# lnkloveating/MediQuery-RAG

Hardware: AMD Instinct MI355X
Metric: queries/s (embed+top-k, k=5, b=256) over 1M×768 corpus; p50 single-query ms (higher is better)
Workload: dtype f32 (exact 3-way bf16 split, fp32 accumulate; exact fp32 top-k)

## Files before the change

mediquery-rag_amd/csrc/encoder.hip:

```cpp
#include <algorithm>
#include <cmath>
#include <cstdlib>
#include <cstring>
#include <memory>
#include <vector>

#include "common.hpp"
#include "gemm_epi.hpp"
#include "gemm_f32.hpp"
#include "gemm_x6p.hpp"

namespace mq {


constexpr int kLnPartW = 96;
constexpr int kLnMaxParts = 8;
struct LnArgs {
  float* stats_out;
  const float* stats_in;
  const float* g;
  const float* b;
  float* xout;
  int ldx;
  int nt;
// ... 94 lines not shown
                                                         const float* __restrict__ W,
                                                         const float* __restrict__ bias,
                                                         const float* __restrict__ resid, int ldr,
                                                         float* __restrict__ out, int ldo, int M,
                                                         int N, int K, LnArgs ln, int rx) {
  __shared__ __attribute__((aligned(16))) float lds[2 * T::STAGE_FLOATS];
  __shared__ float2 ln_st[LN_IN ? 2 * T::BM : 1];
  const int lane = threadIdx.x & 63, wave = __builtin_amdgcn_readfirstlane(threadIdx.x >> 6);
  const int wm = wave / T::WAVES_N, wn = wave % T::WAVES_N;
  const int tiles_n = (N + T::BN - 1) / T::BN, tiles_m = (M + T::BM - 1) / T::BM;
  const int G = gridDim.x, per_xcd = G >> 3;
  const int xslot = (blockIdx.x & 7) * per_xcd + (blockIdx.x >> 3);
  Region rg{0, tiles_m, 0, tiles_n};
  int loc = xslot, wstep = G;
  if (rx > 0) {
    rg = region_of(rx, blockIdx.x & 7, tiles_m, tiles_n);
    loc = blockIdx.x >> 3;
    wstep = per_xcd;
  }
  const int rtiles = rg.rm * rg.rn;
  const int n_tiles = loc < rtiles ? (rtiles - loc + wstep - 1) / wstep : 0;
  const FastDiv tnd(rg.rn);
  auto coords = [&](int i, int& m0, int64_t& n0) {
    const int t = i * wstep + loc;
    const int tr = tnd.div(t);
    m0 = (rg.m_lo + tr) * T::BM;
    n0 = (int64_t)(rg.n_lo + t - tr * rg.rn) * T::BN;
  };
  auto epi = [&](int i, floatx16(&acc)[T::TM][T::TN], float*) {
    int m0;
    int64_t n0l;
    coords(i, m0, n0l);
    const int n0 = (int)n0l;
    if constexpr (EPI == EPI_RESID_STATS) {
      static_assert(T::WN == kLnPartW, "stats partials are per kLnPartW-column wave tile");
      const int wr0 = m0 + wm * T::WM, wc0 = n0 + wn * T::WN;
      const int part = wc0 / T::WN;
      float bv[T::TN];
#pragma unroll
      for (int tn = 0; tn < T::TN; ++tn) bv[tn] = bias[wc0 + tn * 32 + (lane & 31)];
      float rv[T::TM][T::TN][16];
      const bool full = m0 + T::BM <= M;
      const __amdgpu_buffer_rsrc_t ro = __builtin_amdgcn_make_buffer_rsrc(
          (void*)(out + (int64_t)wr0 * ldo + wc0), (short)0, 0x7fffffff, 0x00020000);
      const int ol = (4 * (lane >> 5) * ldo + (lane & 31)) * 4;
      if (full) {
        const __amdgpu_buffer_rsrc_t rr = __builtin_amdgcn_make_buffer_rsrc(
            (void*)(resid + (int64_t)wr0 * ldr + wc0), (short)0, 0x7fffffff, 0x00020000);
        const int rl = (4 * (lane >> 5) * ldr + (lane & 31)) * 4;
#pragma unroll
        for (int tm = 0; tm < T::TM; ++tm)
#pragma unroll
          for (int tn = 0; tn < T::TN; ++tn)
#pragma unroll
            for (int e = 0; e < 16; ++e)
              rv[tm][tn][e] = __uint_as_float(__builtin_amdgcn_raw_buffer_load_b32(
                  rr, rl, (acc_row(tm, e, 0) * ldr + tn * 32) * 4, 0));
      } else {
#pragma unroll
        for (int tm = 0; tm < T::TM; ++tm)
#pragma unroll
          for (int tn = 0; tn < T::TN; ++tn)
#pragma unroll
            for (int e = 0; e < 16; ++e) {
              const int row = min(wr0 + acc_row(tm, e, lane), M - 1);
              rv[tm][tn][e] = resid[(int64_t)row * ldr + wc0 + tn * 32 + (lane & 31)];
// ... 1271 lines not shown
namespace {

struct GemmArgs {
  float* slab;
  size_t slab_floats;
  const float* A;
  int lda;
  const float* W;
  const float* bias;
  const float* resid;
  int ldr;
  float* out;
  int ldo;
  int M, N, K;
  int nt = 0;
  const void* W3 = nullptr;
};

template <class T, int EPI, bool LN_IN = false>
void launch_gemm_t(const GemmArgs& g, int num_cus, hipStream_t s, const LnArgs& ln = LnArgs{}) {
  const int tiles = ((g.M + T::BM - 1) / T::BM) * ((g.N + T::BN - 1) / T::BN);
  const int grid = (std::min(tiles, T::WG_PER_CU * num_cus) + 7) / 8 * 8;
  const int tiles_m = (g.M + T::BM - 1) / T::BM, tiles_n = (g.N + T::BN - 1) / T::BN;
  const int rx = region_pick_rx(tiles_m, tiles_n, (double)T::BM * g.K * 4, (double)T::BN * g.K * 4, grid);
  hipLaunchKernelGGL((gemm_nt_kernel<T, EPI, LN_IN>), dim3(grid), dim3(T::THREADS), 0, s, g.A, g.lda, g.W,
                     g.bias, g.resid, g.ldr, g.out, g.ldo, g.M, g.N, g.K, ln, rx);
}

using GemmBig = F32Tile<2, 2, 2, 2>;
using GemmT96 = F32Tile<4, 1, 1, 3>;
using GemmMid = F32Tile<2, 2, 2, 1>;
using GemmSmall = F32Tile<1, 4, 1, 1>;

using X6Big = F32Tile<2, 2, 2, 2, true>;
using X6T96 = F32Tile<4, 1, 1, 3, true>;
using X6Mid = F32Tile<2, 2, 2, 1, true>;

template <int EPI>
void launch_gemm_tile(const GemmArgs& g, int tile, int num_cus, hipStream_t s) {
  switch (tile) {
    case 0: launch_gemm_t<GemmBig, EPI>(g, num_cus, s); return;
    case 1: launch_gemm_t<GemmT96, EPI>(g, num_cus, s); return;
    case 2: launch_gemm_t<GemmMid, EPI>(g, num_cus, s); return;
    case 5: launch_gemm_t<X6Big, EPI>(g, num_cus, s); return;
    case 6: launch_gemm_t<X6T96, EPI>(g, num_cus, s); return;
    case 7: launch_gemm_t<X6Mid, EPI>(g, num_cus, s); return;
    case 8: launch_gemm_t<F32Tile<4, 2, 1, 3>, EPI>(g, num_cus, s); return;
    case 9: launch_gemm_t<F32Tile<4, 2, 1, 3, true>, EPI>(g, num_cus, s); return;
    default: launch_gemm_t<GemmSmall, EPI>(g, num_cus, s); return;
  }
}

int splitk_factor(const GemmArgs& g, int num_cus, int cap = 16, int tiles_max = 0) {
  if (!g.slab || g.N % 4 != 0) return 0;
  const int64_t tiles = (int64_t)((g.M + 31) / 32) * ((g.N + 127) / 128);
  const int64_t slots = 2 * (int64_t)num_cus;
  if (tiles > (tiles_max > 0 ? tiles_max : num_cus) || g.M > 256) return 0;
  const int slices = g.K / kBK;
  int best = 1;
  for (int s = 1; s <= slices && s <= cap; ++s)
    if (slices % s == 0 && tiles * s <= slots && (size_t)s * g.M * g.N <= g.slab_floats) best = s;
  return best >= 2 ? best : 0;
}

void launch_splitk_gemm(const GemmArgs& g, int S, hipStream_t s) {
  auto go = [&](auto tile) {
    using T = decltype(tile);
    const int tiles = ((g.M + T::BM - 1) / T::BM) * ((g.N + T::BN - 1) / T::BN);
    hipLaunchKernelGGL((gemm_splitk_kernel<T>), dim3(tiles * S), dim3(256), 0, s, g.A, g.lda, g.W, g.M, g.N, g.K,
                       S, g.slab);
  };
  if (g.nt)
    go(F32Tile<1, 4, 1, 1, false, 2, false, 0, true>{});
  else
    go(F32Tile<1, 4, 1, 1>{});
}

template <int EPI>
void launch_splitk(const GemmArgs& g, int S, hipStream_t s) {
  launch_splitk_gemm(g, S, s);
  const int64_t n4 = (int64_t)g.M * g.N / 4;
// ... 980 lines not shown
```

mediquery-rag_amd/csrc/gemm_epi.hpp:

```cpp
#pragma once

#include "gemm_f32.hpp"

namespace mq {

enum Epi { EPI_BIAS = 0, EPI_GELU_ERF = 1, EPI_GELU_TANH = 2, EPI_RESID = 3, EPI_RESID_STATS = 4 };

__device__ __forceinline__ float gelu_erf(float x) {
  const float z = fabsf(x) * 0.70710678118654752f;
  const float t = __builtin_amdgcn_rcpf(fmaf(0.5f, z, 1.0f));
  float p = 0.17087277f;
  p = fmaf(p, t, -0.82215223f);
  p = fmaf(p, t, 1.48851587f);
  p = fmaf(p, t, -1.13520398f);
  p = fmaf(p, t, 0.27886807f);
  p = fmaf(p, t, -0.18628806f);
  p = fmaf(p, t, 0.09678418f);
  p = fmaf(p, t, 0.37409196f);
  p = fmaf(p, t, 1.00002368f);
  p = fmaf(p, t, -1.26551223f);
  const float e = t * __builtin_amdgcn_exp2f(fmaf(-z, z, p) * 1.4426950408889634f);
  return x * (x >= 0.f ? fmaf(-0.5f, e, 1.0f) : 0.5f * e);
}
__device__ __forceinline__ float gelu_tanh(float x) {
// ... 33 lines not shown
    const __amdgpu_buffer_rsrc_t ro = __builtin_amdgcn_make_buffer_rsrc(
        (void*)(out + (int64_t)wr0 * ldo + wc0), (short)0, 0x7fffffff, 0x00020000);
    const int ol = (4 * (lane >> 5) * ldo + (lane & 31)) * 4;
#pragma unroll
    for (int tm = 0; tm < TM; ++tm)
#pragma unroll
      for (int tn = 0; tn < TN; ++tn)
#pragma unroll
        for (int e = 0; e < 16; ++e) {
          float v = epi_apply<EPI>(acc[tm][tn][e] + bv[tn]);
          if constexpr (EPI == EPI_RESID) v += rv[tm][tn][e];
          __builtin_amdgcn_raw_buffer_store_b32(__float_as_uint(v), ro, ol, (acc_row(tm, e, 0) * ldo + tn * 32) * 4, 0);
        }
    return;
  }
#pragma unroll
  for (int tn = 0; tn < TN; ++tn) {
    const int col = wc0 + tn * 32 + (lane & 31);
    if (col >= N) continue;
    const float b = bias[col];
#pragma unroll
    for (int tm = 0; tm < TM; ++tm)
#pragma unroll
      for (int e = 0; e < 16; ++e) {
        const int row = wr0 + acc_row(tm, e, lane);
        if (row >= M) continue;
        float v = epi_apply<EPI>(acc[tm][tn][e] + b);
        if constexpr (EPI == EPI_RESID) v += resid[(int64_t)row * ldr + col];
        out[(int64_t)row * ldo + col] = v;
      }
  }
}

}
```

mediquery-rag_amd/csrc/gemm_f32.hpp:

```cpp
#pragma once

#include "common.hpp"

namespace mq {

constexpr int kBK = 32;
constexpr int kLdsStride = kBK + 4;

typedef __bf16 bf16x8 __attribute__((ext_vector_type(8)));
typedef unsigned uintx4 __attribute__((ext_vector_type(4)));

template <int WAVES_M_, int WAVES_N_, int TM_, int TN_, bool X6_ = false, int PF_ = 2,
          bool BF16_ = false, int BK_ = 0, bool NTB_ = false>
struct F32Tile {
  static constexpr int WAVES_M = WAVES_M_, WAVES_N = WAVES_N_, TM = TM_, TN = TN_;
  static constexpr bool X6 = X6_;
  static constexpr bool NTB = NTB_;
  static constexpr int PF = PF_;
  static constexpr bool BF16 = BF16_;
  static_assert(!(X6 && BF16), "one arithmetic mode");
  static constexpr int WM = TM * 32, WN = TN * 32;
  static constexpr int BM = WAVES_M * WM, BN = WAVES_N * WN;
  static constexpr int THREADS = WAVES_M * WAVES_N * kWave;
  static constexpr int ROWS = BM + BN;
  static constexpr int BK = BK_ ? BK_ : (X6 ? 16 : 32);
  static_assert(BK == 32 || (BK == 16 && !BF16), "slice depth 32, or 16 for the f32 forms");
  static constexpr int F4_PER_ROW = BK / 4;
  static constexpr int ROW_FLOATS = X6 ? 28 : BK + 4;
  static constexpr int TOTAL_F4 = ROWS * F4_PER_ROW;
  static constexpr int LOADS = (TOTAL_F4 + THREADS - 1) / THREADS;
  static constexpr bool PARTIAL = TOTAL_F4 % THREADS != 0;
  static constexpr int STAGE_FLOATS = ROWS * ROW_FLOATS;
  static_assert(THREADS == 256 || THREADS == 512, "4- or 8-wave workgroups");
  static constexpr int WG_PER_CU = THREADS == 256 ? 2 : 1;
  static_assert(BM % 32 == 0 && BN % 32 == 0, "block tile must be a multiple of 32");
  static constexpr bool A_SLOTS = (BM * F4_PER_ROW) % THREADS == 0;
};

__device__ __forceinline__ unsigned pk_bf16(float lo, float hi) {
  unsigned r;
  asm("v_cvt_pk_bf16_f32 %0, %1, %2" : "=v"(r) : "v"(lo), "v"(hi));
  return r;
}
__device__ __forceinline__ float bf16_lo(unsigned p) { return __uint_as_float(p << 16); }
__device__ __forceinline__ float bf16_hi(unsigned p) { return __uint_as_float(p & 0xffff0000u); }

__device__ __forceinline__ void split3(floatx4 x, uint2 (&pl)[3]) {
#pragma unroll
  for (int p = 0; p < 3; ++p) {
    const unsigned a = pk_bf16(x.x, x.y), b = pk_bf16(x.z, x.w);
    pl[p] = make_uint2(a, b);
    if (p < 2) {
      x.x -= bf16_lo(a);
      x.y -= bf16_hi(a);
      x.z -= bf16_lo(b);
      x.w -= bf16_hi(b);
    }
  }
}

template <int V>
struct IC {
  static constexpr int value = V;
};

template <int N, int I = 0, class F>
__device__ __forceinline__ void static_for(F&& f) {
// ... 30 lines not shown
          r[i] = __builtin_bit_cast(floatx4, __builtin_amdgcn_raw_buffer_load_b128(
                                                 rb, min(row - T::BM, blim) * b4 + ch * 16, k0 * 4, T::NTB ? 2 : 0));
      }
      return;
    }
#pragma unroll
    for (int i = 0; i < T::LOADS; ++i) {
      const int f = tid + i * T::THREADS;
      if (T::PARTIAL && i == T::LOADS - 1 && f >= T::TOTAL_F4) break;
      const int row = f / T::F4_PER_ROW, ch = f % T::F4_PER_ROW;
      const float* p;
      const bool a_row = T::A_SLOTS ? i < T::BM * T::F4_PER_ROW / T::THREADS
                                    : f < T::BM * T::F4_PER_ROW;
      if (a_row) {
        p = A + (int64_t)min(m0 + row, M - 1) * lda;
      } else {
        p = B + min(n0 + (int64_t)(row - T::BM), N - 1) * ldb;
      }
      r[i] = *reinterpret_cast<const floatx4*>(p + k0 + ch * 4);
    }
  }

  __device__ __forceinline__ void store(float* stage, int tid) const {
#pragma unroll
    for (int i = 0; i < T::LOADS; ++i) {
      const int f = tid + i * T::THREADS;
      if (T::PARTIAL && i == T::LOADS - 1 && f >= T::TOTAL_F4) break;
      const int row = f / T::F4_PER_ROW, ch = f % T::F4_PER_ROW;
      if constexpr (T::X6) {
        uint2 pl[3];
        split3(r[i], pl);
        char* base = reinterpret_cast<char*>(stage + row * T::ROW_FLOATS) + ch * 8;
#pragma unroll
        for (int p = 0; p < 3; ++p) *reinterpret_cast<uint2*>(base + p * 32) = pl[p];
      } else {
        *reinterpret_cast<floatx4*>(stage + row * T::ROW_FLOATS + ch * 4) = r[i];
      }
    }
  }
};

template <class T>
__device__ __forceinline__ void mma_slice(const float* stage, floatx16 (&acc)[T::TM][T::TN],
                                          int wm, int wn, int lane) {
  const int r = lane & 31, h = lane >> 5;
  if constexpr (T::BF16) {
    const float* as = stage + (wm * T::WM + r) * T::ROW_FLOATS + h * 16;
    const float* bs = stage + (T::BM + wn * T::WN + r) * T::ROW_FLOATS + h * 16;
    bf16x8 a[2][T::TM], b[2][T::TN];
    auto frag = [&](int q, bf16x8(&fa)[T::TM], bf16x8(&fb)[T::TN]) {
#pragma unroll
      for (int tm = 0; tm < T::TM; ++tm)
        fa[tm] = __builtin_bit_cast(bf16x8, *reinterpret_cast<const floatx4*>(as + tm * 32 * T::ROW_FLOATS + q * 4));
#pragma unroll
      for (int tn = 0; tn < T::TN; ++tn)
        fb[tn] = __builtin_bit_cast(bf16x8, *reinterpret_cast<const floatx4*>(bs + tn * 32 * T::ROW_FLOATS + q * 4));
    };
    frag(0, a[0], b[0]);
    __builtin_amdgcn_sched_barrier(0);
#pragma unroll
    for (int q = 0; q < 4; ++q) {
      const int c = q & 1;
      if (q + 1 < 4) frag(q + 1, a[c ^ 1], b[c ^ 1]);
      __builtin_amdgcn_sched_barrier(0);
#pragma unroll
      for (int tm = 0; tm < T::TM; ++tm)
#pragma unroll
        for (int tn = 0; tn < T::TN; ++tn)
          acc[tm][tn] = __builtin_amdgcn_mfma_f32_32x32x16_bf16(a[c][tm], b[c][tn], acc[tm][tn], 0, 0, 0);
      __builtin_amdgcn_sched_barrier(0);
    }
    return;
  }
  if constexpr (T::X6) {
    const char* as = reinterpret_cast<const char*>(stage + (wm * T::WM + r) * T::ROW_FLOATS) + h * 16;
    const char* bs = reinterpret_cast<const char*>(stage + (T::BM + wn * T::WN + r) * T::ROW_FLOATS) + h * 16;
    bf16x8 a[T::TM][3], b[T::TN][3];
#pragma unroll
    for (int tm = 0; tm < T::TM; ++tm)
#pragma unroll
      for (int p = 0; p < 3; ++p)
        a[tm][p] = __builtin_bit_cast(bf16x8, *reinterpret_cast<const uintx4*>(as + tm * 32 * T::ROW_FLOATS * 4 + p * 32));
#pragma unroll
    for (int tn = 0; tn < T::TN; ++tn)
#pragma unroll
      for (int p = 0; p < 3; ++p)
        b[tn][p] = __builtin_bit_cast(bf16x8, *reinterpret_cast<const uintx4*>(bs + tn * 32 * T::ROW_FLOATS * 4 + p * 32));
#pragma unroll
    for (int tm = 0; tm < T::TM; ++tm)
#pragma unroll
      for (int tn = 0; tn < T::TN; ++tn) {
        acc[tm][tn] = __builtin_amdgcn_mfma_f32_32x32x16_bf16(a[tm][2], b[tn][0], acc[tm][tn], 0, 0, 0);
        acc[tm][tn] = __builtin_amdgcn_mfma_f32_32x32x16_bf16(a[tm][1], b[tn][1], acc[tm][tn], 0, 0, 0);
        acc[tm][tn] = __builtin_amdgcn_mfma_f32_32x32x16_bf16(a[tm][0], b[tn][2], acc[tm][tn], 0, 0, 0);
        acc[tm][tn] = __builtin_amdgcn_mfma_f32_32x32x16_bf16(a[tm][1], b[tn][0], acc[tm][tn], 0, 0, 0);
        acc[tm][tn] = __builtin_amdgcn_mfma_f32_32x32x16_bf16(a[tm][0], b[tn][1], acc[tm][tn], 0, 0, 0);
        acc[tm][tn] = __builtin_amdgcn_mfma_f32_32x32x16_bf16(a[tm][0], b[tn][0], acc[tm][tn], 0, 0, 0);
      }
    return;
  }
  constexpr int QN = T::BK / 8;
  const float* as = stage + (wm * T::WM + r) * T::ROW_FLOATS + h * (T::BK / 2);
  const float* bs = stage + (T::BM + wn * T::WN + r) * T::ROW_FLOATS + h * (T::BK / 2);
  floatx4 a[2][T::TM], b[2][T::TN];
// ... 188 lines not shown
```

mediquery-rag_amd/csrc/gemm_x6p.hip:

```cpp
#include <algorithm>

#include "gemm_epi.hpp"
#include "gemm_x6p.hpp"

namespace mq {
namespace {

typedef __attribute__((address_space(3))) void x6p_lds_t;

__device__ __forceinline__ void x6p_glds(const void* base, unsigned voff, unsigned lds_dst) {
  const uint64_t b64 = (uint64_t)(uintptr_t)base;
  base = (const void*)(uintptr_t)(((uint64_t)__builtin_amdgcn_readfirstlane((unsigned)(b64 >> 32)) << 32) |
                                  (unsigned)__builtin_amdgcn_readfirstlane((unsigned)b64));
  unsigned keep;
  asm volatile("s_mov_b32 %0, m0\n\ts_mov_b32 m0, %3\n\ts_nop 0\n\tglobal_load_lds_dwordx4 %1, %2\n\ts_mov_b32 m0, %0"
               : "=&s"(keep)
               : "v"(voff), "s"(base), "s"(__builtin_amdgcn_readfirstlane(lds_dst))
               : "memory");
}

typedef __bf16 bf16x2_t __attribute__((ext_vector_type(2)));
typedef float float2_t __attribute__((ext_vector_type(2)));
__device__ __forceinline__ unsigned cvt_pk_bf16(float lo, float hi) {
  float2_t v;
  v.x = lo;
  v.y = hi;
  return __builtin_bit_cast(unsigned, __builtin_convertvector(v, bf16x2_t));
}
__device__ __forceinline__ void split3v(floatx4 x, uint2 (&pl)[3]) {
#pragma unroll
  for (int p = 0; p < 3; ++p) {
    const unsigned a = cvt_pk_bf16(x.x, x.y), b = cvt_pk_bf16(x.z, x.w);
    pl[p] = make_uint2(a, b);
    if (p < 2) {
      x.x -= bf16_lo(a);
      x.y -= bf16_hi(a);
      x.z -= bf16_lo(b);
      x.w -= bf16_hi(b);
    }
  }
}

#if defined(MQ_X6P_DBG) && !defined(MQ_MEASUREMENT_BUILD)
#error "MQ_X6P_DBG computes wrong results: only a measurement build (-DMQ_MEASUREMENT_BUILD) may set it"
#endif

template <int WAVES_M_, int WAVES_N_, int TM_, int TN_, int NBUF_, int KS_ = 1, int DMAW_ = 8, bool SCHED_ = false,
          int DBG_ = 0, int DSTEP_ = 1, int BR0_ = 0, int PS_ = 4, bool LDR_ = false>
struct X6pTile {
  static constexpr int WAVES_M = WAVES_M_, WAVES_N = WAVES_N_, TM = TM_, TN = TN_, NBUF = NBUF_;
  static constexpr int KS = KS_;
  static constexpr int DMAW = DMAW_;
  static constexpr bool SCHED = SCHED_;
  static constexpr int DSTEP = DSTEP_, BR0 = BR0_, PS = PS_;
  static constexpr int DBG = DBG_;
  static constexpr bool LDR = LDR_;
  static constexpr int NW = WAVES_M * WAVES_N, THREADS = (LDR ? 2 * NW : NW) * 64;
  static constexpr int WM = TM * 32, WN = TN * 32, BM = WAVES_M * WM, BN = WAVES_N * WN;
  static constexpr int A_SUB = BM * 64;
  static constexpr int B_SUB = BN * 96;
  static constexpr int STAGE = KS * (A_SUB + B_SUB);
  static constexpr int NA = BM / 16, NB = BN / 32 * 3;
  static constexpr int NI = KS * (NA + NB);
  static constexpr int CNT_LO = NI / DMAW, REM = NI % DMAW, CNT_HI = CNT_LO + (REM ? 1 : 0);
  static_assert(DMAW == 8 || DMAW == 4, "DMA waves");
  static_assert(!LDR || DMAW == 4, "loader mode: the 4 loader waves issue every DMA");
  static constexpr int AHEAD = KS == 1 ? NBUF : NBUF - 1;
#ifndef MQ_X6P_GM
#define MQ_X6P_GM 4
#endif
  static constexpr int GM = MQ_X6P_GM;
  static_assert(LDR ? NW == 4 : NW == 8, "8-wave workgroups");
  static_assert(!SCHED || (CNT_HI - 1) * DSTEP < TM * TN * 6, "DMAs per k-step slots");
  static_assert(AHEAD >= 2 && NBUF * STAGE <= 160 * 1024, "LDS ring");
};

template <class T, int EPI>
__global__ __launch_bounds__(T::THREADS, 1) void gemm_x6p_kernel(const float* __restrict__ A, int lda,
                                                             const unsigned char* __restrict__ W3,
                                                             const float* __restrict__ bias,
                                                             const float* __restrict__ resid, int ldr,
                                                             float* __restrict__ out, int ldo, int M, int N,
                                                             int K, int rx) {
  __shared__ __attribute__((aligned(1024))) unsigned char lds[T::NBUF * T::STAGE];
  const unsigned lds0 = (unsigned)(uintptr_t)(x6p_lds_t*)lds;
  const int lane = threadIdx.x & 63;
  const int wave = __builtin_amdgcn_readfirstlane(threadIdx.x >> 6);
  const int cw = T::LDR ? wave % T::NW : wave;
  const int wm = cw / T::WAVES_N, wn = cw % T::WAVES_N;
  const int tiles_m = (M + T::BM - 1) / T::BM, tiles_n = (N + T::BN - 1) / T::BN;
  const int total = tiles_m * tiles_n;
  const int G = gridDim.x, per_xcd = G >> 3;
  const int xslot = (blockIdx.x & 7) * per_xcd + (blockIdx.x >> 3);
  int m_lo = 0, rm = tiles_m, n_lo = 0, rn = tiles_n, loc = xslot, wstep = G, rtiles = total;
  if (rx > 0) {
    const Region rg = region_of(rx, blockIdx.x & 7, tiles_m, tiles_n);
    m_lo = rg.m_lo;
    rm = rg.rm;
    n_lo = rg.n_lo;
    rn = rg.rn;
    loc = blockIdx.x >> 3;
    wstep = per_xcd;
    rtiles = rm * rn;
  }
  const int n_tiles = loc < rtiles ? (rtiles - loc + wstep - 1) / wstep : 0;
  if (n_tiles == 0) return;
  const int nk = K >> 4;
  const int nst = nk / T::KS;
  const int S = n_tiles * nst;
  const int nbw = (N + 31) >> 5;
  const int band_tiles = T::GM * rn;
  auto coords = [&](int i, int& m0, int& n0) {
    const int t = i * wstep + loc;
    const int band = t / band_tiles;
    const int gm = min(T::GM, rm - band * T::GM);
    const int w = t - band * band_tiles;
    const int tc = w / gm;
    m0 = (m_lo + band * T::GM + (w - tc * gm)) * T::BM;
    n0 = (n_lo + tc) * T::BN;
  };

  int is_j = 0, is_i = 0, is_kt = 0, is_m0, is_n0;
  coords(0, is_m0, is_n0);
  const unsigned a_chunk = (unsigned)(((lane & 3) ^ ((lane >> 4) & 3)) * 16);
  auto issue_one = [&](int buf, int t) __attribute__((always_inline)) {
    if constexpr (T::DBG & 1) return;
    if constexpr (T::DBG & 64) {
      if (is_j >= T::AHEAD) return;
    }
    const int dw = T::LDR ? wave - T::NW : wave;
    if (dw < 0 || dw >= T::DMAW || (T::REM && t == T::CNT_HI - 1 && dw >= T::REM)) return;
    const unsigned dst = lds0 + (unsigned)(buf * T::STAGE);
    const int ins = dw + t * T::DMAW;
    const int ks = ins / (T::NA + T::NB), in = ins - ks * (T::NA + T::NB);
    const int kt = is_kt + ks;
    if (in < T::NA) {
      if constexpr (T::DBG & 16) return;
      const float* abase = A + (int64_t)is_m0 * lda + kt * 16;
      const unsigned voff = (unsigned)min(16 * in + (lane >> 2), M - 1 - is_m0) * (unsigned)lda * 4u + a_chunk;
      x6p_glds(abase, voff, dst + ks * T::A_SUB + in * 1024);
    } else {
      if constexpr (T::DBG & 32) return;
      const int b = in - T::NA, nbl = b / 3, p = b - nbl * 3;
      const int nbg = min((is_n0 >> 5) + nbl, nbw - 1);
      const unsigned char* wbase = W3 + ((size_t)(nbg * nk + kt) * 3 + p) * 1024;
      x6p_glds(wbase, (unsigned)lane * 16u, dst + T::KS * T::A_SUB + ks * T::B_SUB + b * 1024);
    }
  };
  auto advance = [&]() __attribute__((always_inline)) {
    if (is_j + 1 < S) {
      ++is_j;
      is_kt += T::KS;
      if (is_kt == nk) {
        is_kt = 0;
        ++is_i;
        coords(is_i, is_m0, is_n0);
      }
    }
  };
  auto issue = [&](int buf) __attribute__((always_inline)) {
#pragma unroll
    for (int t = 0; t < T::CNT_HI; ++t) issue_one(buf, t);
    advance();
  };

  const int r = lane & 31, h = lane >> 5, sw = (r >> 2) & 3;
  const unsigned a_lo = (unsigned)((((2 * h) ^ sw) * 16)), a_hi = (unsigned)((((2 * h + 1) ^ sw) * 16));
  struct Frags {
    floatx4 raw[T::TM][2];
    bf16x8 a[T::TM][3], b[T::TN][3];
  };
  auto read_frags = [&](int buf, int ks, Frags& f) __attribute__((always_inline)) {
    if constexpr (T::DBG & 8) return;
    const unsigned char* st = lds + buf * T::STAGE;
#pragma unroll
    for (int tm = 0; tm < T::TM; ++tm) {
      const unsigned char* ar = st + ks * T::A_SUB + (wm * T::WM + tm * 32 + r) * 64;
      f.raw[tm][0] = *reinterpret_cast<const floatx4*>(ar + a_lo);
      f.raw[tm][1] = *reinterpret_cast<const floatx4*>(ar + a_hi);
    }
    const unsigned char* bs = st + T::KS * T::A_SUB + ks * T::B_SUB + lane * 16;
#pragma unroll
    for (int tn = 0; tn < T::TN; ++tn)
#pragma unroll
      for (int p = 0; p < 3; ++p)
        f.b[tn][p] = __builtin_bit_cast(bf16x8, *reinterpret_cast<const uintx4*>(bs + ((wn * T::TN + tn) * 3 + p) * 1024));
  };
  auto split_frags = [&](Frags& f) __attribute__((always_inline)) {
#pragma unroll
    for (int tm = 0; tm < T::TM; ++tm) {
      if constexpr (T::DBG & 2) {
        f.a[tm][0] = __builtin_bit_cast(bf16x8, f.raw[tm][0]);
        f.a[tm][1] = __builtin_bit_cast(bf16x8, f.raw[tm][1]);
        f.a[tm][2] = f.a[tm][0];
        continue;
      }
      uint2 pl[3], ph[3];
      split3v(f.raw[tm][0], pl);
      split3v(f.raw[tm][1], ph);
// ... 103 lines not shown
    constexpr int n = decltype(stages)::value;
    const int dwi = T::LDR ? wave - T::NW : wave;
    if constexpr (T::DBG & 128) {
      if (T::REM && dwi >= 0 && dwi < T::REM)
        asm volatile("s_waitcnt vmcnt(%0)\n\ts_waitcnt lgkmcnt(0)" ::"n"(T::CNT_HI * n) : "memory");
      else
        asm volatile("s_waitcnt vmcnt(%0)\n\ts_waitcnt lgkmcnt(0)" ::"n"(T::CNT_LO * n) : "memory");
      return;
    }
    if (T::REM && dwi >= 0 && dwi < T::REM)
      asm volatile("s_waitcnt vmcnt(%0)" ::"n"(T::CNT_HI * n) : "memory");
    else
      asm volatile("s_waitcnt vmcnt(%0)" ::"n"(T::CNT_LO * n) : "memory");
    __builtin_amdgcn_s_waitcnt(0xC07F);
    asm volatile("s_barrier" ::: "memory");
  };
  zero_acc<T>(acc);

  if constexpr (T::LDR) {
    if (wave >= T::NW) {
#pragma unroll
      for (int d = 0; d < T::AHEAD; ++d) issue(d);
      wait_stages(IC<T::AHEAD - 1>{});
      for (int j = 0; j < S; ++j) {
        wait_stages(IC<T::AHEAD - 2>{});
        issue((j + T::AHEAD) % T::NBUF);
      }
      asm volatile("s_waitcnt vmcnt(0)" ::: "memory");
      return;
    }
  } else {
#pragma unroll
    for (int d = 0; d < T::AHEAD; ++d) issue(d);
  }
  wait_stages(IC<T::AHEAD - 1>{});
  Frags f0 = {}, f1 = {};
  read_frags(0, 0, f0);
  split_frags(f0);
  auto step = [&](int j, Frags& fa, Frags& fb) __attribute__((always_inline)) {
    wait_stages(IC<T::AHEAD - 2>{});
    const int buf = (j + T::AHEAD) % T::NBUF;
    if constexpr (!T::SCHED && !T::LDR) issue(buf);
    static_for<T::KS>([&](auto kc) {
      constexpr int ks = decltype(kc)::value;
      Frags& cur = ks % 2 == 0 ? fa : fb;
      Frags& nxt = ks % 2 == 0 ? fb : fa;
      if constexpr (T::SCHED) {
        constexpr int NM = T::TM * T::TN * 6, NBR = 3 * T::TN, PS = T::PS, NP = 12 * T::TM;
        constexpr int PER = (NP + (NM - PS) - 1) / (NM - PS);
        const int rbuf = ks + 1 < T::KS ? j % T::NBUF : (j + 1) % T::NBUF;
        constexpr int rks = ks + 1 < T::KS ? ks + 1 : 0;
        read_a(rbuf, rks, nxt);
        __builtin_amdgcn_sched_barrier(0);
        static_for<NM>([&](auto ic) {
          constexpr int i = decltype(ic)::value;
          mma_one(cur, i);
          constexpr bool dma_slot = !T::LDR && ks == 0 && i % T::DSTEP == 0 && i / T::DSTEP < T::CNT_HI;
          constexpr int bslot = [] {
            int n = 0;
            for (int k = T::BR0; k < i; ++k)
              if (!(!T::LDR && ks == 0 && k % T::DSTEP == 0 && k / T::DSTEP < T::CNT_HI) || T::DSTEP == 1) ++n;
            return n;
          }();
          if constexpr (i >= T::BR0 && (!dma_slot || T::DSTEP == 1)) {
            if constexpr (2 * bslot < NBR) read_b(rbuf, rks, nxt, 2 * bslot);
            if constexpr (2 * bslot + 1 < NBR) read_b(rbuf, rks, nxt, 2 * bslot + 1);
// ... 28 lines not shown
      if (j + 1 >= S) break;
      step(j + 1, f1, f0);
    }
  }
  asm volatile("s_waitcnt vmcnt(0)" ::: "memory");
}

__global__ __launch_bounds__(256) void split_w3_kernel(const float* __restrict__ W, int N, int K,
                                                       uintx4* __restrict__ w3) {
  const int k8n = K >> 3, np = (N + 31) & ~31;
  const int64_t idx = (int64_t)blockIdx.x * 256 + threadIdx.x;
  if (idx >= (int64_t)np * k8n) return;
  const int n = (int)(idx / k8n), k8 = (int)(idx - (int64_t)n * k8n);
  floatx4 lo = {0.f, 0.f, 0.f, 0.f}, hi = lo;
  if (n < N) {
    lo = *reinterpret_cast<const floatx4*>(W + (int64_t)n * K + 8 * k8);
    hi = *reinterpret_cast<const floatx4*>(W + (int64_t)n * K + 8 * k8 + 4);
  }
  uint2 pl[3], ph[3];
  split3(lo, pl);
  split3(hi, ph);
  const int kb = k8 >> 1, hh = k8 & 1, nb = n >> 5, rr = n & 31;
#pragma unroll
  for (int p = 0; p < 3; ++p) {
    uintx4 v;
    v.x = pl[p].x;
    v.y = pl[p].y;
    v.z = ph[p].x;
    v.w = ph[p].y;
    w3[((int64_t)(nb * (K >> 4) + kb) * 3 + p) * 64 + hh * 32 + rr] = v;
  }
}

using X6p0 = X6pTile<2, 2, 2, 3, 4, 1, 4, true, 0, 1, 0, 6, true>;
using X6p1 = X6pTile<4, 1, 2, 3, 4, 1, 4, true, 0, 1, 0, 6, true>;
using X6p2 = X6pTile<4, 2, 1, 3, 4, 1, 4, true, 0, 2, 1, 6>;
using X6p3 = X6pTile<4, 2, 2, 3, 4, 1, 8, true, 0, 6, 1, 8>;
using X6p4 = X6pTile<2, 2, 2, 3, 3, 2, 4, true, 0, 1, 0, 6, true>;
using X6p5 = X6pTile<2, 2, 2, 3, 4, 1, 4, true, 0, 1, 0, 4, true>;
using X6p6 = X6pTile<2, 2, 2, 3, 5, 1, 4, true, 0, 1, 0, 6, true>;
using X6p7 = X6pTile<2, 2, 1, 3, 4, 1, 4, true, 0, 1, 0, 6, true>;

template <class T, int EPI>
void launch_t(const X6pArgs& g, int num_cus, hipStream_t s) {
  if (g.K % (16 * T::KS) != 0) {
    launch_t<X6pTile<4, 2, 1, 3, 4>, EPI>(g, num_cus, s);
    return;
  }
  const int tiles = ((g.M + T::BM - 1) / T::BM) * ((g.N + T::BN - 1) / T::BN);
  const int grid = (std::min(tiles, num_cus) + 7) / 8 * 8;
  const int tiles_m = (g.M + T::BM - 1) / T::BM, tiles_n = (g.N + T::BN - 1) / T::BN;
  int rx = g.rx;
  if (rx < 0) rx = region_pick_rx(tiles_m, tiles_n, (double)T::BM * g.K * 4, (double)T::BN * g.K * 6, grid);
  if (rx > 0 && (8 % rx != 0 || rx > tiles_n || 8 / rx > tiles_m || grid < 8)) rx = 0;
  hipLaunchKernelGGL((gemm_x6p_kernel<T, EPI>), dim3(grid), dim3(T::THREADS), 0, s, g.A, g.lda,
                     static_cast<const unsigned char*>(g.W3), g.bias, g.resid, g.ldr, g.out, g.ldo, g.M, g.N, g.K, rx);
}

template <int EPI>
void launch_tile(const X6pArgs& g, int tile, int num_cus, hipStream_t s) {
#ifdef MQ_X6P_DBG
  if (tile >= 8) {
    switch (tile) {
      case 8: launch_t<X6pTile<2, 2, 2, 3, 4, 1, 4, true, 64, 1, 0, 6, true>, EPI>(g, num_cus, s); return;
      case 9: launch_t<X6pTile<2, 2, 2, 3, 4, 1, 4, true, 66, 1, 0, 6, true>, EPI>(g, num_cus, s); return;
      case 10: launch_t<X6pTile<2, 2, 2, 3, 4, 1, 4, true, 8, 1, 0, 6, true>, EPI>(g, num_cus, s); return;
      case 11: launch_t<X6pTile<2, 2, 2, 3, 4, 1, 4, true, 74, 1, 0, 6, true>, EPI>(g, num_cus, s); return;
      case 12: launch_t<X6pTile<2, 2, 2, 3, 4, 1, 4, true, 2, 1, 0, 6, true>, EPI>(g, num_cus, s); return;
      case 13: launch_t<X6pTile<2, 2, 2, 3, 4, 1, 4, true, 256, 1, 0, 6, true>, EPI>(g, num_cus, s); return;
      case 14: launch_t<X6pTile<2, 2, 2, 3, 4, 1, 4, true, 512, 1, 0, 6, true>, EPI>(g, num_cus, s); return;
      default: launch_t<X6pTile<2, 2, 2, 3, 4, 1, 4, true, 128, 1, 0, 6, true>, EPI>(g, num_cus, s); return;
    }
  }
#endif
  switch (tile) {
    case 1: launch_t<X6p1, EPI>(g, num_cus, s); return;
    case 2: launch_t<X6p2, EPI>(g, num_cus, s); return;
    case 3: launch_t<X6p3, EPI>(g, num_cus, s); return;
    case 4: launch_t<X6p4, EPI>(g, num_cus, s); return;
    case 5: launch_t<X6p5, EPI>(g, num_cus, s); return;
    case 6: launch_t<X6p6, EPI>(g, num_cus, s); return;
    case 7: launch_t<X6p7, EPI>(g, num_cus, s); return;
    default: launch_t<X6p0, EPI>(g, num_cus, s); return;
  }
}

}

void launch_split_w3(const float* W, int N, int K, void* w3, hipStream_t s) {
  const int64_t n = (int64_t)((N + 31) & ~31) * (K >> 3);
  hipLaunchKernelGGL(split_w3_kernel, dim3((unsigned)((n + 255) / 256)), dim3(256), 0, s, W, N, K,
                     static_cast<uintx4*>(w3));
}

int x6p_pick_tile(int M, int N, int num_cus) {
  auto rounds = [&](int bm, int bn) {
    const int64_t tiles = (int64_t)((M + bm - 1) / bm) * ((N + bn - 1) / bn);
    return (tiles + num_cus - 1) / num_cus;
  };
  return rounds(256, 96) < rounds(128, 192) ? 1 : 0;
}

void launch_gemm_x6p(const X6pArgs& g, int epi, int tile, int num_cus, hipStream_t s) {
  if (tile < 0) {
    tile = x6p_pick_tile(g.M, g.N, num_cus);
    const int64_t t0 = (int64_t)((g.M + 127) / 128) * ((g.N + 191) / 192);
    if (g.K <= 768 && g.N <= 768 && t0 <= num_cus && t0 * 2 > num_cus) tile = 7;
  }
  switch (epi) {
    case EPI_GELU_ERF: launch_tile<EPI_GELU_ERF>(g, tile, num_cus, s); return;
    case EPI_GELU_TANH: launch_tile<EPI_GELU_TANH>(g, tile, num_cus, s); return;
    case EPI_RESID: launch_tile<EPI_RESID>(g, tile, num_cus, s); return;
    default: launch_tile<EPI_BIAS>(g, tile, num_cus, s); return;
  }
}

}

extern "C" {

int64_t mq_debug_w3_bytes(int N, int K) { return N > 0 && K > 0 && K % 16 == 0 ? (int64_t)mq::w3_bytes(N, K) : -1; }

int mq_debug_split_w3(const float* W, int N, int K, void* w3, void* stream) {
  using namespace mq;
  clear_error();
  MQ_CHECK_ARG(W && w3, "NULL buffer");
  MQ_CHECK_ARG(N > 0 && K > 0 && K % 16 == 0, "bad shape N=%d K=%d", N, K);
  launch_split_w3(W, N, K, w3, (hipStream_t)stream);
  MQ_HIP(hipGetLastError());
  return MQ_OK;
}

int mq_debug_gemm_x6p(const float* A, const void* W3, const float* bias, const float* resid, float* out, int M,
                      int N, int K, int epi, int tile, void* stream) {
  using namespace mq;
  clear_error();
  MQ_CHECK_ARG(A && W3 && bias && out && (epi != EPI_RESID || resid), "NULL buffer");
  MQ_CHECK_ARG(M > 0 && N > 0 && K > 0 && K % 32 == 0, "bad shape M=%d N=%d K=%d", M, N, K);
  const int rx = tile >= 100 ? tile / 100 - 1 : -1;
  if (tile >= 100) tile %= 100;
  MQ_CHECK_ARG(epi >= 0 && epi <= 3 && tile >= -1 && tile <= 15 && rx <= 8, "bad epi/tile");
  int dev = 0, cus = 256;
  (void)hipGetDevice(&dev);
  (void)hipDeviceGetAttribute(&cus, hipDeviceAttributeMultiprocessorCount, dev);
  X6pArgs g{A, K, W3, bias, resid, N, out, N, M, N, K};
  g.rx = rx;
  launch_gemm_x6p(g, epi, tile, cus, (hipStream_t)stream);
  MQ_HIP(hipGetLastError());
  return MQ_OK;
}

}
```

Before: 33320.

## Switch split-f32 GEMMs to 16x16x32 bf16 MFMA with 32-deep stages

Adds a 16x16x32 bf16 MFMA path for the 3-way split f32 GEMMs, in both the generic F32Tile kernel and the pipelined X6p kernel. It uses 32-deep K slices, reorganised LDS rows, a new LDS swizzle, and a 16-row epilogue store helper. The default X6p tiles become these 16x16 variants with KS=2 and fewer ring buffers, and the old 32x32 forms are kept as tiles 16/17. The small-shape override to tile 7 is also removed. The aim is higher MFMA throughput and better interleaving of the split and the DMA. The cost is one workgroup per CU for the F32Tile variants, and more register pressure from the extra scheduling complexity.

```diff
diff --git a/mediquery-rag_amd/csrc/encoder.hip b/mediquery-rag_amd/csrc/encoder.hip
--- a/mediquery-rag_amd/csrc/encoder.hip
+++ b/mediquery-rag_amd/csrc/encoder.hip
@@ -150,6 +150,19 @@
     int64_t n0l;
     coords(i, m0, n0l);
     const int n0 = (int)n0l;
+    if constexpr (T::M16) {
+      static_assert(EPI != EPI_RESID_STATS, "no LayerNorm partials on the 16x16x32 tiles");
+      floatx4 a4[2 * T::TM][2 * T::TN];
+#pragma unroll
+      for (int m = 0; m < 2 * T::TM; ++m)
+#pragma unroll
+        for (int n = 0; n < 2 * T::TN; ++n)
+#pragma unroll
+          for (int e = 0; e < 4; ++e) a4[m][n][e] = acc[m >> 1][n >> 1][4 * (2 * (m & 1) + (n & 1)) + e];
+      store_wave_tile16<EPI, 2 * T::TM, 2 * T::TN>(a4, m0 + wm * T::WM, n0 + wn * T::WN, M, N, bias, resid, ldr, out,
+                                                   ldo, lane);
+      return;
+    }
     if constexpr (EPI == EPI_RESID_STATS) {
       static_assert(T::WN == kLnPartW, "stats partials are per kLnPartW-column wave tile");
       const int wr0 = m0 + wm * T::WM, wc0 = n0 + wn * T::WN;
@@ -1487,9 +1500,10 @@
 using GemmMid = F32Tile<2, 2, 2, 1>;
 using GemmSmall = F32Tile<1, 4, 1, 1>;
 
-using X6Big = F32Tile<2, 2, 2, 2, true>;
-using X6T96 = F32Tile<4, 1, 1, 3, true>;
-using X6Mid = F32Tile<2, 2, 2, 1, true>;
+using X6Big = F32Tile<2, 2, 2, 2, true, 2, false, 0, false, true>;
+using X6T96 = F32Tile<4, 1, 1, 3, true, 2, false, 0, false, true>;
+using X6Mid = F32Tile<2, 2, 2, 1, true, 2, false, 0, false, true>;
+using X6W192 = F32Tile<4, 2, 1, 3, true, 2, false, 0, false, true>;
 
 template <int EPI>
 void launch_gemm_tile(const GemmArgs& g, int tile, int num_cus, hipStream_t s) {
@@ -1501,7 +1515,7 @@
     case 6: launch_gemm_t<X6T96, EPI>(g, num_cus, s); return;
     case 7: launch_gemm_t<X6Mid, EPI>(g, num_cus, s); return;
     case 8: launch_gemm_t<F32Tile<4, 2, 1, 3>, EPI>(g, num_cus, s); return;
-    case 9: launch_gemm_t<F32Tile<4, 2, 1, 3, true>, EPI>(g, num_cus, s); return;
+    case 9: launch_gemm_t<X6W192, EPI>(g, num_cus, s); return;
     default: launch_gemm_t<GemmSmall, EPI>(g, num_cus, s); return;
   }
 }
diff --git a/mediquery-rag_amd/csrc/gemm_epi.hpp b/mediquery-rag_amd/csrc/gemm_epi.hpp
--- a/mediquery-rag_amd/csrc/gemm_epi.hpp
+++ b/mediquery-rag_amd/csrc/gemm_epi.hpp
@@ -89,4 +89,59 @@
   }
 }
 
+template <int EPI, int MB, int NB>
+__device__ __forceinline__ void store_wave_tile16(floatx4 (&acc)[MB][NB], int wr0, int wc0, int M, int N,
+                                                  const float* __restrict__ bias, const float* __restrict__ resid,
+                                                  int ldr, float* __restrict__ out, int ldo, int lane) {
+  const int c = lane & 15, g = lane >> 4;
+  if (wr0 + MB * 16 <= M && wc0 + NB * 16 <= N) {
+    float bv[NB];
+#pragma unroll
+    for (int n = 0; n < NB; ++n) bv[n] = bias[wc0 + n * 16 + c];
+    const __amdgpu_buffer_rsrc_t rr = __builtin_amdgcn_make_buffer_rsrc(
+        (void*)(resid + (EPI == EPI_RESID ? (int64_t)wr0 * ldr + wc0 : 0)), (short)0, 0x7fffffff, 0x00020000);
+    const int rl = (4 * g * ldr + c) * 4;
+    const __amdgpu_buffer_rsrc_t ro = __builtin_amdgcn_make_buffer_rsrc(
+        (void*)(out + (int64_t)wr0 * ldo + wc0), (short)0, 0x7fffffff, 0x00020000);
+    const int ol = (4 * g * ldo + c) * 4;
+#pragma unroll
+    for (int m = 0; m < MB; ++m) {
+      float rv[NB][4];
+      if constexpr (EPI == EPI_RESID) {
+#pragma unroll
+        for (int n = 0; n < NB; ++n)
+#pragma unroll
+          for (int e = 0; e < 4; ++e)
+            rv[n][e] = __uint_as_float(
+                __builtin_amdgcn_raw_buffer_load_b32(rr, rl, ((m * 16 + e) * ldr + n * 16) * 4, 0));
+      }
+#pragma unroll
+      for (int n = 0; n < NB; ++n)
+#pragma unroll
+        for (int e = 0; e < 4; ++e) {
+          float v = epi_apply<EPI>(acc[m][n][e] + bv[n]);
+          if constexpr (EPI == EPI_RESID) v += rv[n][e];
+          __builtin_amdgcn_raw_buffer_store_b32(__float_as_uint(v), ro, ol, ((m * 16 + e) * ldo + n * 16) * 4, 0);
+        }
+    }
+    return;
+  }
+#pragma unroll
+  for (int n = 0; n < NB; ++n) {
+    const int col = wc0 + n * 16 + c;
+    if (col >= N) continue;
+    const float b = bias[col];
+#pragma unroll
+    for (int m = 0; m < MB; ++m)
+#pragma unroll
+      for (int e = 0; e < 4; ++e) {
+        const int row = wr0 + m * 16 + 4 * g + e;
+        if (row >= M) continue;
+        float v = epi_apply<EPI>(acc[m][n][e] + b);
+        if constexpr (EPI == EPI_RESID) v += resid[(int64_t)row * ldr + col];
+        out[(int64_t)row * ldo + col] = v;
+      }
+  }
 }
+
+}
diff --git a/mediquery-rag_amd/csrc/gemm_f32.hpp b/mediquery-rag_amd/csrc/gemm_f32.hpp
--- a/mediquery-rag_amd/csrc/gemm_f32.hpp
+++ b/mediquery-rag_amd/csrc/gemm_f32.hpp
@@ -11,10 +11,12 @@
 typedef unsigned uintx4 __attribute__((ext_vector_type(4)));
 
 template <int WAVES_M_, int WAVES_N_, int TM_, int TN_, bool X6_ = false, int PF_ = 2,
-          bool BF16_ = false, int BK_ = 0, bool NTB_ = false>
+          bool BF16_ = false, int BK_ = 0, bool NTB_ = false, bool M16_ = false>
 struct F32Tile {
   static constexpr int WAVES_M = WAVES_M_, WAVES_N = WAVES_N_, TM = TM_, TN = TN_;
   static constexpr bool X6 = X6_;
+  static constexpr bool M16 = M16_;
+  static_assert(!M16 || X6, "the 16x16x32 form is a split-f32 option");
   static constexpr bool NTB = NTB_;
   static constexpr int PF = PF_;
   static constexpr bool BF16 = BF16_;
@@ -23,16 +25,16 @@
   static constexpr int BM = WAVES_M * WM, BN = WAVES_N * WN;
   static constexpr int THREADS = WAVES_M * WAVES_N * kWave;
   static constexpr int ROWS = BM + BN;
-  static constexpr int BK = BK_ ? BK_ : (X6 ? 16 : 32);
+  static constexpr int BK = BK_ ? BK_ : (X6 && !M16 ? 16 : 32);
   static_assert(BK == 32 || (BK == 16 && !BF16), "slice depth 32, or 16 for the f32 forms");
   static constexpr int F4_PER_ROW = BK / 4;
-  static constexpr int ROW_FLOATS = X6 ? 28 : BK + 4;
+  static constexpr int ROW_FLOATS = X6 ? (M16 ? 52 : 28) : BK + 4;
   static constexpr int TOTAL_F4 = ROWS * F4_PER_ROW;
   static constexpr int LOADS = (TOTAL_F4 + THREADS - 1) / THREADS;
   static constexpr bool PARTIAL = TOTAL_F4 % THREADS != 0;
   static constexpr int STAGE_FLOATS = ROWS * ROW_FLOATS;
   static_assert(THREADS == 256 || THREADS == 512, "4- or 8-wave workgroups");
-  static constexpr int WG_PER_CU = THREADS == 256 ? 2 : 1;
+  static constexpr int WG_PER_CU = THREADS == 256 && !M16 ? 2 : 1;
   static_assert(BM % 32 == 0 && BN % 32 == 0, "block tile must be a multiple of 32");
   static constexpr bool A_SLOTS = (BM * F4_PER_ROW) % THREADS == 0;
 };
@@ -129,7 +131,7 @@
         split3(r[i], pl);
         char* base = reinterpret_cast<char*>(stage + row * T::ROW_FLOATS) + ch * 8;
 #pragma unroll
-        for (int p = 0; p < 3; ++p) *reinterpret_cast<uint2*>(base + p * 32) = pl[p];
+        for (int p = 0; p < 3; ++p) *reinterpret_cast<uint2*>(base + p * (T::BK * 2)) = pl[p];
       } else {
         *reinterpret_cast<floatx4*>(stage + row * T::ROW_FLOATS + ch * 4) = r[i];
       }
@@ -167,6 +169,39 @@
           acc[tm][tn] = __builtin_amdgcn_mfma_f32_32x32x16_bf16(a[c][tm], b[c][tn], acc[tm][tn], 0, 0, 0);
       __builtin_amdgcn_sched_barrier(0);
     }
+    return;
+  }
+  if constexpr (T::X6 && T::M16) {
+    const int c = lane & 15, kq = lane >> 4;
+    const char* as = reinterpret_cast<const char*>(stage + (wm * T::WM + c) * T::ROW_FLOATS) + kq * 16;
+    const char* bs = reinterpret_cast<const char*>(stage + (T::BM + wn * T::WN + c) * T::ROW_FLOATS) + kq * 16;
+    bf16x8 a[2 * T::TM][3], b[2 * T::TN][3];
+#pragma unroll
+    for (int m = 0; m < 2 * T::TM; ++m)
+#pragma unroll
+      for (int p = 0; p < 3; ++p)
+        a[m][p] = __builtin_bit_cast(bf16x8, *reinterpret_cast<const uintx4*>(as + m * 16 * T::ROW_FLOATS * 4 + p * 64));
+#pragma unroll
+    for (int n = 0; n < 2 * T::TN; ++n)
+#pragma unroll
+      for (int p = 0; p < 3; ++p)
+        b[n][p] = __builtin_bit_cast(bf16x8, *reinterpret_cast<const uintx4*>(bs + n * 16 * T::ROW_FLOATS * 4 + p * 64));
+#pragma unroll
+    for (int m = 0; m < 2 * T::TM; ++m)
+#pragma unroll
+      for (int n = 0; n < 2 * T::TN; ++n) {
+        floatx16& full = acc[m >> 1][n >> 1];
+        const int q = 4 * (2 * (m & 1) + (n & 1));
+        floatx4 d = {full[q], full[q + 1], full[q + 2], full[q + 3]};
+        d = __builtin_amdgcn_mfma_f32_16x16x32_bf16(a[m][2], b[n][0], d, 0, 0, 0);
+        d = __builtin_amdgcn_mfma_f32_16x16x32_bf16(a[m][1], b[n][1], d, 0, 0, 0);
+        d = __builtin_amdgcn_mfma_f32_16x16x32_bf16(a[m][0], b[n][2], d, 0, 0, 0);
+        d = __builtin_amdgcn_mfma_f32_16x16x32_bf16(a[m][1], b[n][0], d, 0, 0, 0);
+        d = __builtin_amdgcn_mfma_f32_16x16x32_bf16(a[m][0], b[n][1], d, 0, 0, 0);
+        d = __builtin_amdgcn_mfma_f32_16x16x32_bf16(a[m][0], b[n][0], d, 0, 0, 0);
+#pragma unroll
+        for (int e = 0; e < 4; ++e) full[q + e] = d[e];
+      }
     return;
   }
   if constexpr (T::X6) {
diff --git a/mediquery-rag_amd/csrc/gemm_x6p.hip b/mediquery-rag_amd/csrc/gemm_x6p.hip
--- a/mediquery-rag_amd/csrc/gemm_x6p.hip
+++ b/mediquery-rag_amd/csrc/gemm_x6p.hip
@@ -19,6 +19,8 @@
                : "memory");
 }
 
+__device__ __forceinline__ int a_swz(int q) { return q ^ (q >> 1); }
+
 typedef __bf16 bf16x2_t __attribute__((ext_vector_type(2)));
 typedef float float2_t __attribute__((ext_vector_type(2)));
 __device__ __forceinline__ unsigned cvt_pk_bf16(float lo, float hi) {
@@ -46,7 +48,8 @@
 #endif
 
 template <int WAVES_M_, int WAVES_N_, int TM_, int TN_, int NBUF_, int KS_ = 1, int DMAW_ = 8, bool SCHED_ = false,
-          int DBG_ = 0, int DSTEP_ = 1, int BR0_ = 0, int PS_ = 4, bool LDR_ = false>
+          int DBG_ = 0, int DSTEP_ = 1, int BR0_ = 0, int PS_ = 4, bool LDR_ = false, bool M16_ = false,
+          bool DEEP_ = false>
 struct X6pTile {
   static constexpr int WAVES_M = WAVES_M_, WAVES_N = WAVES_N_, TM = TM_, TN = TN_, NBUF = NBUF_;
   static constexpr int KS = KS_;
@@ -55,6 +58,7 @@
   static constexpr int DSTEP = DSTEP_, BR0 = BR0_, PS = PS_;
   static constexpr int DBG = DBG_;
   static constexpr bool LDR = LDR_;
+  static constexpr bool M16 = M16_, DEEP = DEEP_;
   static constexpr int NW = WAVES_M * WAVES_N, THREADS = (LDR ? 2 * NW : NW) * 64;
   static constexpr int WM = TM * 32, WN = TN * 32, BM = WAVES_M * WM, BN = WAVES_N * WN;
   static constexpr int A_SUB = BM * 64;
@@ -65,13 +69,15 @@
   static constexpr int CNT_LO = NI / DMAW, REM = NI % DMAW, CNT_HI = CNT_LO + (REM ? 1 : 0);
   static_assert(DMAW == 8 || DMAW == 4, "DMA waves");
   static_assert(!LDR || DMAW == 4, "loader mode: the 4 loader waves issue every DMA");
-  static constexpr int AHEAD = KS == 1 ? NBUF : NBUF - 1;
+  static constexpr int AHEAD = KS == 1 || (M16 && DEEP) ? NBUF : NBUF - 1;
+  static_assert(!M16 || (KS == 2 && SCHED), "16x16x32 body: slot-scheduled 32-deep stages");
+  static_assert(!DEEP || M16, "DEEP is a 16x16x32 option");
 #ifndef MQ_X6P_GM
 #define MQ_X6P_GM 4
 #endif
   static constexpr int GM = MQ_X6P_GM;
   static_assert(LDR ? NW == 4 : NW == 8, "8-wave workgroups");
-  static_assert(!SCHED || (CNT_HI - 1) * DSTEP < TM * TN * 6, "DMAs per k-step slots");
+  static_assert(!SCHED || (CNT_HI - 1) * DSTEP < TM * TN * 6 * (M16 ? 4 : 1), "DMAs per k-step slots");
   static_assert(AHEAD >= 2 && NBUF * STAGE <= 160 * 1024, "LDS ring");
 };
 
@@ -122,7 +128,7 @@
 
   int is_j = 0, is_i = 0, is_kt = 0, is_m0, is_n0;
   coords(0, is_m0, is_n0);
-  const unsigned a_chunk = (unsigned)(((lane & 3) ^ ((lane >> 4) & 3)) * 16);
+  const unsigned a_chunk = (unsigned)(((lane & 3) ^ a_swz((lane >> 4) & 3)) * 16);
   auto issue_one = [&](int buf, int t) __attribute__((always_inline)) {
     if constexpr (T::DBG & 1) return;
     if constexpr (T::DBG & 64) {
@@ -164,7 +170,7 @@
     advance();
   };
 
-  const int r = lane & 31, h = lane >> 5, sw = (r >> 2) & 3;
+  const int r = lane & 31, h = lane >> 5, sw = a_swz((r >> 2) & 3);
   const unsigned a_lo = (unsigned)((((2 * h) ^ sw) * 16)), a_hi = (unsigned)((((2 * h + 1) ^ sw) * 16));
   struct Frags {
     floatx4 raw[T::TM][2];
@@ -334,6 +340,107 @@
   } else {
 #pragma unroll
     for (int d = 0; d < T::AHEAD; ++d) issue(d);
+  }
+  if constexpr (T::M16) {
+    constexpr int MB = 2 * T::TM, NB16 = 2 * T::TN, RS = NB16 * 6, NM16 = MB * RS, NSUB = 28;
+    static_assert(RS >= NSUB + 4, "a region holds one block's split and its raw reads");
+    const int c = lane & 15, kq = lane >> 4, hq = kq & 1, sw16 = a_swz((c >> 2) & 3);
+    const unsigned a_base = (unsigned)((kq >> 1) * T::A_SUB + (wm * T::WM + c) * 64);
+    const unsigned a_lo16 = a_base + (unsigned)(((2 * hq) ^ sw16) * 16);
+    const unsigned a_hi16 = a_base + (unsigned)(((2 * hq + 1) ^ sw16) * 16);
+    const unsigned b_base =
+        (unsigned)(T::KS * T::A_SUB + (kq >> 1) * T::B_SUB + wn * T::TN * 3 * 1024 + hq * 512 + c * 16);
+    floatx4 acc4[MB][NB16];
+    uintx4 au[MB][3];
+    bf16x8 bw[NB16][3];
+    floatx4 raw[2];
+    auto rd_raw = [&](const unsigned char* st, int m, int half) __attribute__((always_inline)) {
+      raw[half] = *reinterpret_cast<const floatx4*>(st + m * 1024 + (half ? a_hi16 : a_lo16));
+    };
+    auto rd_b = [&](const unsigned char* st, int n, int p) __attribute__((always_inline)) {
+      bw[n][p] = __builtin_bit_cast(
+          bf16x8, *reinterpret_cast<const uintx4*>(st + b_base + ((n >> 1) * 3 + p) * 1024 + (n & 1) * 256));
+    };
+    auto sub = [&](int m, int q) __attribute__((always_inline)) {
+      const int half = q / 14, rq = q % 14;
+      const int p = rq < 12 ? rq / 6 : 2, part = rq < 12 ? (rq % 6) / 3 : rq - 12, op = rq < 12 ? rq % 3 : 0;
+      floatx4& x = raw[half];
+      if (op == 0) {
+        unsigned u = cvt_pk_bf16(x[2 * part], x[2 * part + 1]);
+        asm volatile("" : "+v"(u));
+        au[m][p][2 * half + part] = u;
+      } else {
+        const unsigned u = au[m][p][2 * half + part];
+        if (op == 1)
+          x[2 * part] -= bf16_lo(u);
+        else
+          x[2 * part + 1] -= bf16_hi(u);
+        asm volatile("" : "+v"(x));
+      }
+    };
+    auto zero4 = [&]() __attribute__((always_inline)) {
+#pragma unroll
+      for (int m = 0; m < MB; ++m)
+#pragma unroll
+        for (int n = 0; n < NB16; ++n) acc4[m][n] = floatx4{0.f, 0.f, 0.f, 0.f};
+    };
+    zero4();
+    wait_stages(IC<T::AHEAD - 1>{});
+#pragma unroll
+    for (int m = 0; m < MB; ++m) {
+      rd_raw(lds, m, 0);
+      rd_raw(lds, m, 1);
+      if (m < MB - 1) {
+#pragma unroll
+        for (int q = 0; q < NSUB; ++q) sub(m, q);
+      }
+    }
+#pragma unroll
+    for (int n = 0; n < NB16; ++n)
+#pragma unroll
+      for (int p = 0; p < 3; ++p) rd_b(lds, n, p);
+    int rb = 1 % T::NBUF;
+    int ib = T::AHEAD % T::NBUF;
+    for (int j = 0; j < S; ++j) {
+      if constexpr (!T::LDR) {
+        wait_stages(IC<T::AHEAD - 2>{});
+      } else {
+        if constexpr (T::DEEP) __builtin_amdgcn_s_waitcnt(0xC07F);
+        asm volatile("s_barrier" ::: "memory");
+      }
+      const unsigned char* st = lds + rb * T::STAGE;
+      static_for<NM16>([&](auto ic) {
+        constexpr int i = decltype(ic)::value;
+        constexpr int m = i / RS, w = i % RS, n = w / 6, term = w % 6;
+        constexpr int pa = term == 0 ? 2 : term == 1 || term == 3 ? 1 : 0;
+        constexpr int pb = term == 0 || term >= 3 ? (term == 4 ? 1 : 0) : term == 1 ? 1 : 2;
+        acc4[m][n] = __builtin_amdgcn_mfma_f32_16x16x32_bf16(__builtin_bit_cast(bf16x8, au[m][pa]), bw[n][pb],
+                                                             acc4[m][n], 0, 0, 0);
+        if constexpr (w >= 2 && w < 2 + NSUB) sub((m + MB - 1) % MB, w - 2);
+        if constexpr (w == 2 + NSUB || w == 3 + NSUB) rd_raw(st, m, w - 2 - NSUB);
+        if constexpr (m == MB - 1 && term == 2) rd_b(st, n, 2);
+        if constexpr (m == MB - 1 && term == 4) rd_b(st, n, 1);
+        if constexpr (m == MB - 1 && term == 5) rd_b(st, n, 0);
+        if constexpr (!T::LDR && i % T::DSTEP == 0 && i / T::DSTEP < T::CNT_HI) issue_one(ib, i / T::DSTEP);
+        __builtin_amdgcn_sched_barrier(0);
+      });
+      if constexpr (!T::LDR) {
+        advance();
+        ib = ib + 1 == T::NBUF ? 0 : ib + 1;
+      }
+      rb = rb + 1 == T::NBUF ? 0 : rb + 1;
+      if (++c_st == nst) {
+        c_st = 0;
+        int m0, n0;
+        coords(c_i, m0, n0);
+        store_wave_tile16<EPI, MB, NB16>(acc4, m0 + wm * T::WM, n0 + wn * T::WN, M, N, bias, resid, ldr, out, ldo,
+                                         lane);
+        zero4();
+        ++c_i;
+      }
+    }
+    if constexpr (!T::LDR) asm volatile("s_waitcnt vmcnt(0)" ::: "memory");
+    return;
   }
   wait_stages(IC<T::AHEAD - 1>{});
   Frags f0 = {}, f1 = {};
@@ -428,14 +535,16 @@
   }
 }
 
-using X6p0 = X6pTile<2, 2, 2, 3, 4, 1, 4, true, 0, 1, 0, 6, true>;
-using X6p1 = X6pTile<4, 1, 2, 3, 4, 1, 4, true, 0, 1, 0, 6, true>;
-using X6p2 = X6pTile<4, 2, 1, 3, 4, 1, 4, true, 0, 2, 1, 6>;
-using X6p3 = X6pTile<4, 2, 2, 3, 4, 1, 8, true, 0, 6, 1, 8>;
-using X6p4 = X6pTile<2, 2, 2, 3, 3, 2, 4, true, 0, 1, 0, 6, true>;
-using X6p5 = X6pTile<2, 2, 2, 3, 4, 1, 4, true, 0, 1, 0, 4, true>;
-using X6p6 = X6pTile<2, 2, 2, 3, 5, 1, 4, true, 0, 1, 0, 6, true>;
-using X6p7 = X6pTile<2, 2, 1, 3, 4, 1, 4, true, 0, 1, 0, 6, true>;
+using X6p0 = X6pTile<2, 2, 2, 3, 3, 2, 4, true, 0, 1, 0, 6, true, true>;
+using X6p1 = X6pTile<4, 1, 2, 3, 3, 2, 4, true, 0, 1, 0, 6, true, true>;
+using X6p2 = X6pTile<4, 2, 1, 3, 3, 2, 4, true, 0, 2, 1, 6, false, true>;
+using X6p3 = X6pTile<4, 2, 2, 3, 2, 2, 8, true, 0, 6, 1, 8, false, true, true>;
+using X6p4 = X6pTile<2, 2, 2, 3, 3, 2, 4, true, 0, 1, 0, 6, true, true, true>;
+using X6p5 = X6pTile<2, 2, 1, 3, 3, 2, 4, true, 0, 1, 0, 6, true, true, true>;
+using X6p6 = X6pTile<4, 1, 2, 3, 3, 2, 4, true, 0, 1, 0, 6, true, true, true>;
+using X6p7 = X6pTile<2, 2, 1, 3, 3, 2, 4, true, 0, 1, 0, 6, true, true>;
+using X6p16 = X6pTile<2, 2, 2, 3, 4, 1, 4, true, 0, 1, 0, 6, true>;
+using X6p17 = X6pTile<2, 2, 1, 3, 4, 1, 4, true, 0, 1, 0, 6, true>;
 
 template <class T, int EPI>
 void launch_t(const X6pArgs& g, int num_cus, hipStream_t s) {
@@ -477,6 +586,8 @@
     case 5: launch_t<X6p5, EPI>(g, num_cus, s); return;
     case 6: launch_t<X6p6, EPI>(g, num_cus, s); return;
     case 7: launch_t<X6p7, EPI>(g, num_cus, s); return;
+    case 16: launch_t<X6p16, EPI>(g, num_cus, s); return;
+    case 17: launch_t<X6p17, EPI>(g, num_cus, s); return;
     default: launch_t<X6p0, EPI>(g, num_cus, s); return;
   }
 }
@@ -500,8 +611,6 @@
 void launch_gemm_x6p(const X6pArgs& g, int epi, int tile, int num_cus, hipStream_t s) {
   if (tile < 0) {
     tile = x6p_pick_tile(g.M, g.N, num_cus);
-    const int64_t t0 = (int64_t)((g.M + 127) / 128) * ((g.N + 191) / 192);
-    if (g.K <= 768 && g.N <= 768 && t0 <= num_cus && t0 * 2 > num_cus) tile = 7;
   }
   switch (epi) {
     case EPI_GELU_ERF: launch_tile<EPI_GELU_ERF>(g, tile, num_cus, s); return;
@@ -535,7 +644,7 @@
   MQ_CHECK_ARG(M > 0 && N > 0 && K > 0 && K % 32 == 0, "bad shape M=%d N=%d K=%d", M, N, K);
   const int rx = tile >= 100 ? tile / 100 - 1 : -1;
   if (tile >= 100) tile %= 100;
-  MQ_CHECK_ARG(epi >= 0 && epi <= 3 && tile >= -1 && tile <= 15 && rx <= 8, "bad epi/tile");
+  MQ_CHECK_ARG(epi >= 0 && epi <= 3 && tile >= -1 && tile <= 17 && rx <= 8, "bad epi/tile");
   int dev = 0, cus = 256;
   (void)hipGetDevice(&dev);
   (void)hipDeviceGetAttribute(&cus, hipDeviceAttributeMultiprocessorCount, dev);
```

After: 37390, median of 6. 12.2% higher.
